# Cyan4973/FiniteStateEntropy

Hardware: NVIDIA H100
Metric: encode+decode GB/s (uncompressed) per GPU on 32 KB blocks; bit-exact vs ref (higher is better)
Workload: dtype u8

## Files before the change

finitestateentropy_b200/csrc/huf_decode.cu:

```cuda
#include "common.cuh"
#include "launchers.h"
#include "huf_dev.cuh"
#include "launch_util.cuh"
#include <cstdlib>
#include <type_traits>

namespace fseb {
namespace hufd {

#ifndef FSEB200_HUFD_HEAD
#define FSEB200_HUFD_HEAD 1
#endif

constexpr int G = 64;
constexpr int THREADS = 4 * G;
constexpr int NWARPS = THREADS / 32;
constexpr int RW = 8;
constexpr u32 RING_BYTES = RW * THREADS * 4;
__host__ __device__ constexpr int threads_for(int ns) { return ns * G; }
__host__ __device__ constexpr u32 ring_bytes(int ns) { return RW * threads_for(ns) * 4; }
constexpr u32 NOERR = 0xFFFFFFFFu;
constexpr unsigned FULL = 0xFFFFFFFFu;
constexpr u32 MIN_ROWS = 160;
constexpr u32 PARK_RANKEND = 128, PARK_LISTSTART = 142;
constexpr u64 HDR_STREAM_MAX = 1ull << 20;

struct __align__(16) Facts {
    u32 bid[G];
    u32 status[G];
    u32 hsize[G];
    u16 dOff[G];
    u16 cut[G];
    u8  tlog[G];
    u8  mbits[G];
    u8  kind[G];
    u8  hard[G];
};
template <int NW>
struct BuildScratchT {
    u8  weights[NW][256];
    u8  sorted[NW][256];
    u32 rankStats[NW][HUF_MAX_TLOG + 1];
    u16 rankRun[NW][HUF_MAX_TLOG + 2];
    u16 rankEnd[NW][HUF_MAX_TLOG + 2];
    u16 listStart[NW][HUF_MAX_TLOG + 2];
};
typedef BuildScratchT<NWARPS> BuildScratch;
static_assert(sizeof(BuildScratch) <= RING_BYTES, "build scratch must fit in the ring");
static_assert(sizeof(BuildScratchT<threads_for(1) / 32>) <= ring_bytes(1), "build scratch must fit in the 1X ring");
static_assert(sizeof(Facts) == 1280, "Facts layout");
constexpr u32 NOBLOCK = 0xFFFFFFFFu;

constexpr u32 STAGE_WARP_BYTES = 32 * 32;
__host__ __device__ constexpr u32 smem_bytes(u32 rows, bool staged, int ns = 4)
{
    return rows * (G * 2) + ring_bytes(ns) + (u32)sizeof(Facts) + (staged ? (u32)(threads_for(ns) / 32) * STAGE_WARP_BYTES : 0u);
}

__device__ __forceinline__ u32 lds_u16(u32 addr) { u16 v; asm volatile("ld.shared.u16 %0, [%1];" : "=h"(v) : "r"(addr)); return v; }
__device__ __forceinline__ u32 lds_u32(u32 addr) { u32 v; asm volatile("ld.shared.u32 %0, [%1];" : "=r"(v) : "r"(addr)); return v; }
__device__ __forceinline__ void sts_u32(u32 addr, u32 v) { asm volatile("st.shared.u32 [%0], %1;" :: "r"(addr), "r"(v) : "memory"); }

__device__ __forceinline__ u32 head_symbols(const u8* outp) { return (u32)(0ull - reinterpret_cast<u64>(outp)) & 31u; }

__device__ __forceinline__ u32 canon_cell(const u16* rankEnd, const u16* listStart, const u8* sorted, u32 idx, u32 tl)
{
    u32 w = 1;
    while (idx >= rankEnd[w]) w++;
    u32 const first = (w == 1) ? 0u : rankEnd[w - 1];
    u32 const k = listStart[w] + ((idx - first) >> (w - 1));
    return (tl + 1 - w) | ((u32)sorted[k] << 8);
}

__device__ u64 warp_huf_read_stats(u8* weights, u32* rankStats, u32* nbSymPtr, u32* tlPtr, const u8* in, u64 srcSize, unsigned lane)
{
    if (!srcSize) return err(E_SRC_WRONG);
    u64 iSize = in[0], oSize;
    if (iSize >= 128) {
        oSize = iSize - 127;
        iSize = (oSize + 1) / 2;
        if (iSize + 1 > srcSize) return err(E_SRC_WRONG);
        if (oSize >= 256) return err(E_CORRUPT);
        for (u32 k = lane; k < (u32)iSize; k += 32) { u8 const v = in[1 + k]; weights[2 * k] = v >> 4; weights[2 * k + 1] = v & 15; }
    } else {
        if (iSize + 1 > srcSize) return err(E_SRC_WRONG);
        oSize = 0;
        if (lane == 0) oSize = d_huf_read_weights_fse(weights, 256, in, iSize);
        oSize = __shfl_sync(FULL, oSize, 0);
        if (is_err(oSize)) return oSize;
    }
    if (lane <= HUF_MAX_TLOG) rankStats[lane] = 0;
    __syncwarp();
    u32 total = 0; bool bad = false;
    for (u32 n = lane; n < (u32)oSize; n += 32) {
        u32 const w = weights[n];
        if (w >= HUF_MAX_TLOG) bad = true;
        else { atomicAdd(&rankStats[w], 1u); total += (1u << w) >> 1; }
    }
    if (__any_sync(FULL, bad)) return err(E_CORRUPT);
    #pragma unroll
    for (int d = 16; d; d >>= 1) total += __shfl_xor_sync(FULL, total, d);
    if (total == 0) return err(E_CORRUPT);
    u32 const tl = hibit(total) + 1;
    if (tl > HUF_MAX_TLOG) return err(E_CORRUPT);
    u32 const rest = (1u << tl) - total;
    u32 const lastW = hibit(rest) + 1;
    if ((1u << hibit(rest)) != rest) return err(E_CORRUPT);
    __syncwarp();
    if (lane == 0) { weights[oSize] = (u8)lastW; rankStats[lastW]++; }
    __syncwarp();
    if ((rankStats[1] < 2) || (rankStats[1] & 1)) return err(E_CORRUPT);
    *tlPtr = tl;
    *nbSymPtr = (u32)(oSize + 1);
    return iSize + 1;
}

template <bool EXT = false, class BS>
__device__ void setup_block(u16* tbl, Facts& fx, BS& bs, u32 rows, int blk, const u8* csrc, u64 csize, int warp)
{
    unsigned const lane = lane_id();
    u8* const weights = bs.weights[warp];
    u8* const sorted = bs.sorted[warp];
    u16* const rankEnd = bs.rankEnd[warp];
    u16* const listStart = bs.listStart[warp];
    u32 nbSym = 0, tl = 0, M = 0, cut = 0, nRows = 0;
    u64 h = warp_huf_read_stats(weights, bs.rankStats[warp], &nbSym, &tl, csrc, csize, lane);
    if (lane == 0) {
        if (!is_err(h) && tl > HUF_MAX_TLOG) h = err(E_TLOG_TOO_LARGE);
        if (!EXT && !is_err(h) && h >= csize) h = err(E_SRC_WRONG);
        if (!is_err(h)) {
            u32 acc = 0, pos = 0;
            rankEnd[0] = 0; listStart[0] = 0;
            for (u32 w = 1; w <= tl; w++) {
                listStart[w] = (u16)pos; bs.rankRun[warp][w] = (u16)pos;
                pos += bs.rankStats[warp][w];
                acc += bs.rankStats[warp][w] << (w - 1);
                rankEnd[w] = (u16)(acc > 0xFFFF ? 0xFFFF : acc);
            }
            rankEnd[tl] = (u16)(1u << tl);
            rankEnd[tl + 1] = 0xFFFF;
            M = tl; cut = 0; nRows = 1u << tl;
            for (u32 m = (tl > 10 ? 10 : tl - 1); m >= 4 && m < tl; m--) {
                u32 const g = 1u << (tl - m);
                u32 const T = rankEnd[tl - m];
                u32 const c = (T + g - 1) & ~(g - 1);
                u32 const r = c + (1u << m) - (c >> (tl - m));
                if (r < nRows) { nRows = r; M = m; cut = c; }
            }
            fx.hard[blk] = (u8)(nRows > rows);
            fx.tlog[blk] = (u8)tl;
            fx.mbits[blk] = (u8)M;
            fx.cut[blk] = (u16)cut;
            fx.dOff[blk] = (u16)(M < tl ? cut - (cut >> (tl - M)) : 0);
            fx.hsize[blk] = EXT ? 0u : (u32)h;
        } else {
            atomicMin(&fx.status[blk], (u32)(0u << 8 | (u32)(0 - h)));
        }
    }
    h = __shfl_sync(FULL, h, 0);
    if (is_err(h)) return;
    M = __shfl_sync(FULL, M, 0); cut = __shfl_sync(FULL, cut, 0); nRows = __shfl_sync(FULL, nRows, 0);
    __syncwarp();
    for (u32 base = 0; base < nbSym; base += 32) {
        u32 const s = base + lane;
        u32 const w = (s < nbSym) ? weights[s] : 0u;
        u32 const peers = __match_any_sync(FULL, w);
        if (w) sorted[bs.rankRun[warp][w] + __popc(peers & ((1u << lane) - 1))] = (u8)s;
        __syncwarp();
        if (w && (peers >> lane) == 1u) bs.rankRun[warp][w] = (u16)(bs.rankRun[warp][w] + __popc(peers));
        __syncwarp();
    }
    u16* const col = tbl + blk;
    if (nRows <= rows) {
        u32 const D = (M < tl) ? cut - (cut >> (tl - M)) : 0u;
        for (u32 row = lane; row < nRows; row += 32) {
            u32 const x = (row < cut || M == tl) ? row : ((row - D) << (tl - M));
            col[row * G] = (u16)canon_cell(rankEnd, listStart, sorted, x, tl);
        }
    } else {
        for (u32 r = lane; r < 128; r += 32) col[r * G] = (u16)(sorted[2 * r] | (sorted[2 * r + 1] << 8));
        if (lane < HUF_MAX_TLOG + 2) { col[(PARK_RANKEND + lane) * G] = rankEnd[lane]; col[(PARK_LISTSTART + lane) * G] = listStart[lane]; }
    }
    __syncwarp();
}

template <bool PASS_A, class Geo, int NS>
__global__ void __launch_bounds__(NS * G, NS == 4 ? 4 : 5)
huf_decode_kernel(Geo g, u8* __restrict__ dst, const u8* __restrict__ cbuf, const u64* __restrict__ csizes,
                  u64* __restrict__ results, const u8* __restrict__ orig, u32 flags, u32 gEff, u32 rows,
                  const u32* __restrict__ list, const u32* __restrict__ listCount, u32* __restrict__ deferList, u32* __restrict__ deferCount)
{
    static_assert(NS == 4 || NS == 1, "4X or 1X");
    constexpr int NT = threads_for(NS);
    constexpr int NW = NT / 32;
    constexpr u32 RB = ring_bytes(NS);
    extern __shared__ __align__(16) unsigned char smem_raw[];
    unsigned char* const ringRaw = smem_raw;
    BuildScratchT<NW>& bs = *reinterpret_cast<BuildScratchT<NW>*>(ringRaw);
    Facts& fx = *reinterpret_cast<Facts*>(ringRaw + RB);
    u16* const tbl = reinterpret_cast<u16*>(smem_raw + RB + sizeof(Facts));
    int const tid = threadIdx.x, warp = tid >> 5, lane = tid & 31;
    u32 const blk0 = blockIdx.x * gEff;
    u32 const nWork = list ? *listCount : g.nBlocks;
    if (blk0 >= nWork) return;
    u32 const blkEnd = min(blk0 + gEff, nWork);

    if (tid < G) { fx.bid[tid] = (blk0 + tid < blkEnd) ? (list ? list[blk0 + tid] : blk0 + tid) : NOBLOCK; fx.status[tid] = NOERR; fx.kind[tid] = 3; fx.hsize[tid] = 0; fx.tlog[tid] = 0; fx.mbits[tid] = 0; fx.cut[tid] = 0; fx.dOff[tid] = 0; fx.hard[tid] = 0; }
    __syncthreads();

    for (int j = warp; j < G; j += NW) {
        u32 const b = fx.bid[j];
        if (b == NOBLOCK) continue;
        u64 const n = dec_len(g, b);
        u64 const cs = dec_csize(g, csizes, b);
        int kind;
        if constexpr (std::is_same_v<Geo, HeaderDescs>) {
            if (n > HUF_BLOCK_MAX) { kind = 3; if (lane == 0) dec_out(g, results, b) = err(E_SRC_WRONG); }
            else kind = 0;
        } else if constexpr (!Geo::DESCS) {
            if (flags & 1u) kind = 0;
            else if (is_err(cs)) { kind = 3; if (lane == 0) results[b] = cs; }
            else if (cs == 0) { kind = orig ? 1 : 3; if (lane == 0) results[b] = orig ? n : 0; }
            else if (n == 0) { kind = 3; if (lane == 0) results[b] = err(E_DST_TOO_SMALL); }
            else if (cs > n) { kind = 3; if (lane == 0) results[b] = err(E_CORRUPT); }
            else if (cs == n) kind = 1;
            else if (cs == 1) kind = 2;
            else kind = 0;
        } else {
            if (n == 0) { kind = 3; if (lane == 0) dec_out(g, results, b) = err(E_DST_TOO_SMALL); }
            else if (n > HUF_BLOCK_MAX) { kind = 3; if (lane == 0) dec_out(g, results, b) = err(E_SRC_WRONG); }
            else if (cs > n) { kind = 3; if (lane == 0) dec_out(g, results, b) = err(E_CORRUPT); }
            else if (cs == n) kind = 1;
            else if (cs == 1) kind = 2;
            else kind = 0;
        }
        if (lane == 0) fx.kind[j] = (u8)kind;
        if (kind == 0) {
            if constexpr (std::is_same_v<Geo, HeaderDescs>) {
                u64 const hb = g.hdrSize[b];
                if (hb) setup_block<true>(tbl, fx, bs, rows, j, g.hdr[b], hb, warp);
                else setup_block(tbl, fx, bs, rows, j, dec_src(g, cbuf, b), cs, warp);
            } else setup_block(tbl, fx, bs, rows, j, dec_src(g, cbuf, b), cs, warp);
            if (deferList && fx.hard[j] && fx.status[j] == NOERR) {
                if (lane == 0) { deferList[atomicAdd(deferCount, 1u)] = b; fx.kind[j] = 3; }
            }
        }
    }
    __syncthreads();

    int const col = 2 * lane + (NS == 4 ? warp >> 2 : warp);
    int const strm = (NS == 4) ? warp & 3 : 0;
    u32 const b = fx.bid[col];
    bool const live = (b != NOBLOCK) && fx.kind[col] == 0 && fx.status[col] == NOERR;
    u32 const n = live ? dec_len(g, b) : 0;
    u32 const seg = (NS == 4) ? (n + 3) / 4 : n;
    u32 segLen = 0;
    u8* outp = (Geo::DESCS && !live) ? nullptr : dec_dst(g, dst, b) + (u64)strm * seg;
    const u8* blockStart = nullptr;
    u64 chunkTop = 0;
    u32 expectBits = 0;
    u32 c0 = 0;
    u32 const tl = fx.tlog[col];

    if (live) {
        const u8* const cs0 = dec_src(g, cbuf, b);
        u64 const cs = dec_csize(g, csizes, b);
        blockStart = cs0;
        const u8* const pay = cs0 + fx.hsize[col];
        u64 const psize = cs - fx.hsize[col];
        u32 code = 0;
        constexpr bool HDR = std::is_same_v<Geo, HeaderDescs>;
        bool tooLong = false;
        if constexpr (NS == 4) {
            if (psize < 10) code = E_CORRUPT;
            else if (3 * seg > n) code = E_CORRUPT;
            else {
                u32 const l1 = rd16(pay), l2 = rd16(pay + 2), l3 = rd16(pay + 4);
                if ((u64)l1 + l2 + l3 + 6 > psize) code = E_CORRUPT;
                else {
                    u32 const l4 = (u32)(psize - 6 - l1 - l2 - l3);
                    u32 const off = 6 + (strm > 0 ? l1 : 0) + (strm > 1 ? l2 : 0) + (strm > 2 ? l3 : 0);
                    u32 const len = strm == 0 ? l1 : strm == 1 ? l2 : strm == 2 ? l3 : l4;
                    u64 const len64 = (HDR && strm == 3) ? psize - 6 - l1 - l2 - l3 : len;
                    if (HDR ? len64 < 1 : len < 1) code = E_SRC_WRONG;
                    else {
                        u8 const last = HDR ? pay[off + len64 - 1] : pay[off + len - 1];
                        if (last == 0) code = (HDR ? len64 >= 8 : len >= 8) ? E_GENERIC : E_CORRUPT;
                        else if (HDR && len64 > HDR_STREAM_MAX) tooLong = true;
                        else {
                            u64 const sBegin = (u64)(pay + off);
                            u64 const e = sBegin + len;
                            chunkTop = ((e - 1) & ~31ull) + 32;
                            c0 = (u32)(8 * (chunkTop - e)) + (8 - hibit(last));
                            expectBits = (u32)(8 * (chunkTop - sBegin));
                            segLen = (strm < 3) ? seg : n - 3 * seg;
                        }
                    }
                }
            }
        } else if (HDR && (psize < 1 || psize > HDR_STREAM_MAX)) {
            if (psize < 1) code = E_SRC_WRONG;
            else if (pay[psize - 1] == 0) code = E_GENERIC;
            else tooLong = true;
        } else {
            u32 const len = (u32)psize;
            u8 const last = pay[len - 1];
            if (last == 0) code = (len >= 8) ? E_GENERIC : E_CORRUPT;
            else {
                u64 const sBegin = (u64)pay;
                u64 const e = sBegin + len;
                chunkTop = ((e - 1) & ~31ull) + 32;
                c0 = (u32)(8 * (chunkTop - e)) + (8 - hibit(last));
                expectBits = (u32)(8 * (chunkTop - sBegin));
                segLen = n;
            }
        }
        if (code) atomicMin(&fx.status[col], (u32)((1u + strm) << 8 | code));
        if (tooLong) atomicMin(&fx.status[col], (u32)(5u << 8 | E_CORRUPT));
    }
    __syncthreads();
    bool const go = live && fx.status[col] == NOERR;
    if (!go) segLen = 0;

    u32 const ringLane = (u32)__cvta_generic_to_shared(ringRaw) + tid * 4;
    u32 pLimit;
    if constexpr (Geo::DESCS) pLimit = go ? (u32)((chunkTop - dec_floor(g, cbuf, blockStart)) >> 5) - 1u : 0u;
    else pLimit = go ? (u32)((chunkTop - (reinterpret_cast<u64>(cbuf) & ~31ull)) >> 5) - 1u : 0u;
    u32 m0 = 0, m1 = 0, m2 = 0, m3 = 0, m4 = 0, m5 = 0, m6 = 0, m7 = 0;
    constexpr bool staged = PASS_A;
    auto load_pair = [&](u32 pr) {
        u64 const a = chunkTop - 32ull * (min(pr, pLimit) + 1);
        if (!staged) {
            asm volatile("ld.global.nc.v4.b32 {%0, %1, %2, %3}, [%8];\n\t"
                         "ld.global.nc.v4.b32 {%4, %5, %6, %7}, [%8+16];"
                         : "=r"(m0), "=r"(m1), "=r"(m2), "=r"(m3), "=r"(m4), "=r"(m5), "=r"(m6), "=r"(m7) : "l"(a));
            asm volatile("prefetch.global.L2 [%0];" :: "l"(chunkTop - 32ull * (min(pr + 2, pLimit) + 1)));
            return;
        }
        u32 const dead = (a & 127) == 0;
        asm volatile("{\n\t.reg .pred p;\n\t.reg .b64 pol;\n\tsetp.ne.u32 p, %9, 0;\n\t"
                     "createpolicy.fractional.L2::evict_first.b64 pol, 1.0;\n\t"
                     "@p ld.global.nc.L2::cache_hint.v4.b32 {%0, %1, %2, %3}, [%8], pol;\n\t"
                     "@p ld.global.nc.L2::cache_hint.v4.b32 {%4, %5, %6, %7}, [%8+16], pol;\n\t"
                     "@!p ld.global.nc.v4.b32 {%0, %1, %2, %3}, [%8];\n\t"
                     "@!p ld.global.nc.v4.b32 {%4, %5, %6, %7}, [%8+16];\n\t}"
                     : "=r"(m0), "=r"(m1), "=r"(m2), "=r"(m3), "=r"(m4), "=r"(m5), "=r"(m6), "=r"(m7) : "l"(a), "r"(dead));
        {
            if ((a & 127) == 96 && pr + 11 <= pLimit) asm volatile("cp.async.bulk.prefetch.L2.global [%0], 128;" :: "l"(a - 352));
        }
    };

    u32 w0 = 0, w1 = 0, w2 = 0, r = 0;
    u32 kBase = 0;
    u32 q = 0;
    auto store_next = [&]() {
        u32 const a = ringLane + (q & 1) * (4 * NT * 4);
        bool const lowHalf = (q & 1) != 0;
        sts_u32(a, lowHalf ? m3 : m7); sts_u32(a + NT * 4, lowHalf ? m2 : m6);
        sts_u32(a + 2 * NT * 4, lowHalf ? m1 : m5); sts_u32(a + 3 * NT * 4, lowHalf ? m0 : m4);
        q++;
        if (!(q & 1)) load_pair(q >> 1);
    };
    auto unread = [&]() -> u32 { return 4 * q - kBase - (r >> 5); };
    auto top_up = [&](u32 threshold) { if (unread() <= threshold) store_next(); };

    if (go) {
        u32 const k0 = c0 >> 5;
        r = c0 & 31;
        q = 2 * (k0 >> 3);
        load_pair(q >> 1);
        store_next(); store_next();
        kBase = k0;
        auto fetch_word = [&]() -> u32 {
            u32 const v = lds_u32(ringLane + (kBase & 7) * (NT * 4));
            kBase++;
            if (!(kBase & 7)) store_next();
            return v;
        };
        w0 = fetch_word(); w1 = fetch_word(); w2 = fetch_word();
        top_up(4);
    }

    u32 const tblCol = (u32)__cvta_generic_to_shared(tbl) + col * 2;
    u32 const M = fx.mbits[col];
    u32 const shX = 32 - (tl ? tl : 1);
    u32 const shY = 32 - (M ? M : 1);
    int const dOff = (int)fx.dOff[col];
    u32 const tblColD = tblCol + (u32)dOff * (G * 2);
    bool const hardBlk = fx.hard[col] != 0;

    static_assert(NT * 4 % 32 == 0 && (NT * 4 & (NT * 4 - 1)) == 0, "slot stride: a power of two, a multiple of 32");
    u32 const tid4 = tid * 4;
    u32 const ringBase = (u32)__cvta_generic_to_shared(ringRaw);
    u32 const slotBias = kBase * (NT * 4);
    u32 hi = __funnelshift_l(w1, w0, r), lo = __funnelshift_l(w2, w1, r);
#define HUFD_LOOKUP(E, H) do { \
        int const a_ = (int)((H) >> shX) - dOff; \
        int const y_ = (int)((H) >> shY); \
        E = lds_u16((u32)min(a_, y_) * (G * 2) + tblColD); \
    } while (0)
#define HUFD_ADVANCE(PACKED) do { \
        u32 const rOld_ = r; \
        r = __dp4a((u32)(PACKED), 0x00010001u, r); \
        u32 const ra_ = ((rOld_ * (NT * 4 / 32u) + slotBias) & ((RW - 1) * NT * 4)) | tid4; \
        asm volatile("{\n\t.reg .pred p;\n\t.reg .b32 t;\n\t" \
                     "xor.b32 t, %4, %5;\n\tand.b32 t, t, 32;\n\tsetp.ne.u32 p, t, 0;\n\t" \
                     "@p mov.b32 %0, %1;\n\t@p mov.b32 %1, %2;\n\t@p ld.shared.u32 %2, [%3];\n\t}" \
                     : "+r"(w0), "+r"(w1), "+r"(w2) : "r"(ringBase + ra_), "r"(r), "r"(rOld_) : "memory"); \
        hi = __funnelshift_l(w1, w0, r); lo = __funnelshift_l(w2, w1, r); \
    } while (0)

    u32 pos = 0;
    constexpr bool withHead = Geo::DESCS && FSEB200_HUFD_HEAD;
    bool const fastOk = withHead ? go && !hardBlk && segLen >= head_symbols(outp) + 32u
                                 : go && !hardBlk && ((reinterpret_cast<u64>(outp) & 31) == 0);
    u32 const headN = (withHead && fastOk) ? head_symbols(outp) : 0u;
    if constexpr (withHead) {
        for (u32 i = 0; i < headN; i++) {
            if ((i & 7) == 0) top_up(4);
            u32 e;
            HUFD_LOOKUP(e, hi);
            HUFD_ADVANCE(e);
            outp[pos++] = (u8)(e >> 8);
        }
    }
    u32 const nIter = fastOk ? (segLen - headN) >> 5 : 0u;
    u32 const nIterW = __reduce_max_sync(FULL, nIter);
    u32 const stageW = (u32)__cvta_generic_to_shared(tbl) + rows * (G * 2) + (u32)warp * STAGE_WARP_BYTES;
    for (u32 it = 0; it < nIterW; it++) {
        bool const act = it < nIter;
        u32 o[8];
        if (act) {
            #pragma unroll
            for (int h = 0; h < 8; h++) {
                if ((h & 3) == 0) top_up(4);
                else if ((h & 3) == 2 && __builtin_expect(__any_sync(__activemask(), unread() <= 3), 0)) top_up(3);
                u32 e0, e1, e2, e3, hi1;
                HUFD_LOOKUP(e0, hi); hi1 = __funnelshift_l(lo, hi, e0); HUFD_LOOKUP(e1, hi1);
                u32 const p01 = e0 | (e1 << 16);
                HUFD_ADVANCE(p01);
                HUFD_LOOKUP(e2, hi); hi1 = __funnelshift_l(lo, hi, e2); HUFD_LOOKUP(e3, hi1);
                u32 const p23 = e2 | (e3 << 16);
                HUFD_ADVANCE(p23);
                o[h] = __byte_perm(p01, p23, 0x7531);
            }
        }
        if (!staged) {
            if (act)
                asm volatile("st.global.v4.b32 [%0], {%1, %2, %3, %4};\n\tst.global.v4.b32 [%0+16], {%5, %6, %7, %8};"
                             :: "l"(outp + pos), "r"(o[0]), "r"(o[1]), "r"(o[2]), "r"(o[3]), "r"(o[4]), "r"(o[5]), "r"(o[6]), "r"(o[7]) : "memory");
            if (act) pos += 32;
            continue;
        }
        if (act)
            asm volatile("st.shared.v4.b32 [%0], {%1, %2, %3, %4};\n\tst.shared.v4.b32 [%0+16], {%5, %6, %7, %8};"
                         :: "r"(stageW + (u32)lane * 32), "r"(o[0]), "r"(o[1]), "r"(o[2]), "r"(o[3]), "r"(o[4]), "r"(o[5]), "r"(o[6]), "r"(o[7]) : "memory");
        __syncwarp();
        u64 const dstHere = reinterpret_cast<u64>(outp + pos);
        u32 const o32 = (u32)dstHere - pos;
        bool const lineDone = ((((o32 + pos) | 127u) + 1u) - o32) <= headN + nIter * 32u;
        u32 const flags = (act ? 1u : 0u) | (lineDone ? 2u : 0u);
        #pragma unroll
        for (int k = 0; k < 2; k++) {
            int const src = k * 16 + (lane >> 1);
            u32 const half = (u32)(lane & 1) * 16;
            u64 const q = __shfl_sync(FULL, dstHere, src);
            u32 const srcFlags = __shfl_sync(FULL, flags, src);
            u32 x0, x1, x2, x3;
            asm volatile("ld.shared.v4.b32 {%0, %1, %2, %3}, [%4];" : "=r"(x0), "=r"(x1), "=r"(x2), "=r"(x3) : "r"(stageW + (u32)src * 32 + half));
            u32 const keep = (srcFlags & 2u) && ((q + half) & 127) < 96;
            if (srcFlags & 1u)
                asm volatile("{\n\t.reg .pred p;\n\t.reg .b64 pl, pf;\n\tsetp.ne.u32 p, %5, 0;\n\t"
                             "createpolicy.fractional.L2::evict_last.b64 pl, 1.0;\n\t"
                             "createpolicy.fractional.L2::evict_first.b64 pf, 1.0;\n\t"
                             "@p st.global.L2::cache_hint.v4.b32 [%0], {%1, %2, %3, %4}, pl;\n\t"
                             "@!p st.global.L2::cache_hint.v4.b32 [%0], {%1, %2, %3, %4}, pf;\n\t}"
                             :: "l"(q + half), "r"(x0), "r"(x1), "r"(x2), "r"(x3), "r"(keep) : "memory");
        }
        __syncwarp();
        if (act) pos += 32;
    }
    if (pos < segLen) {
        const u16* const colp = tbl + col;
        auto parked_cell = [&](u32 idx) -> u32 {
            u32 w = 1;
            while (idx >= colp[(PARK_RANKEND + w) * G]) w++;
            u32 const first = (w == 1) ? 0u : colp[(PARK_RANKEND + w - 1) * G];
            u32 const k = colp[(PARK_LISTSTART + w) * G] + ((idx - first) >> (w - 1));
            return (tl + 1 - w) | (((colp[(k >> 1) * G] >> (8 * (k & 1))) & 0xFFu) << 8);
        };
        u32 cnt = 0;
        while (pos < segLen) {
            if ((cnt++ & 7) == 0) top_up(4);
            u32 e;
            if (hardBlk) e = parked_cell(hi >> (32 - tl));
            else HUFD_LOOKUP(e, hi);
            HUFD_ADVANCE(e);
            outp[pos++] = (u8)(e >> 8);
        }
    }
#undef HUFD_LOOKUP
#undef HUFD_ADVANCE

    if (go) {
        u64 const fetched = 4ull * q - unread();
        u64 const consumed = 32ull * (fetched - 3) + (r & 31);
        if (consumed != (u64)expectBits) atomicMin(&fx.status[col], (u32)(5u << 8 | E_CORRUPT));
    }
    __syncthreads();
    if (tid < G) {
        u32 const bb = fx.bid[tid];
        if (bb != NOBLOCK && fx.kind[tid] == 0) {
            u32 const st = fx.status[tid];
            u64 rv = (st == NOERR) ? (u64)dec_len(g, bb) : err(st & 0xFF);
            if ((st >> 8) == 5u && ((flags & 2u) || (!(flags & 1u) && d_huf_select_decoder(dec_len(g, bb), dec_csize(g, csizes, bb))))) rv = HUF_X2_PENDING;
            dec_out(g, results, bb) = rv;
        }
    }
    for (int j = 0; j < G; j++) {
        int const kd = fx.kind[j];
        if (kd != 1 && kd != 2) continue;
        u32 const bb = fx.bid[j];
        u32 const nn = dec_len(g, bb);
        u64 const cs = dec_csize(g, csizes, bb);
        u8* const o = dec_dst(g, dst, bb);
        if (kd == 2) { u8 const v = dec_src(g, cbuf, bb)[0]; for (u32 i = tid; i < nn; i += NT) o[i] = v; }
        else {
            const u8* const s = (cs == 0) ? dec_orig(g, orig, bb) : dec_src(g, cbuf, bb);
            for (u32 i = tid; i < nn; i += NT) o[i] = s[i];
        }
        if (tid == 0) dec_out(g, results, bb) = nn;
    }
}

constexpr int FORM_THREADS = 256;
struct HufMixedSplit {
    const u64* dstCap; const u8* single; u64* cap4; u64* cap1; const u64* res1; u64* result;
    u32 nBlocks;
};

__global__ void __launch_bounds__(FORM_THREADS) huf_mixed_split_kernel(HufMixedSplit g)
{
    u64 const b = (u64)blockIdx.x * FORM_THREADS + threadIdx.x;
    if (b >= g.nBlocks) return;
    u64 const n = g.dstCap[b], none = (u64)HUF_BLOCK_MAX + 1;
    bool const one = g.single[b] != 0;
    g.cap4[b] = one ? none : n;
    g.cap1[b] = one ? n : none;
}

__global__ void __launch_bounds__(FORM_THREADS) huf_mixed_merge_kernel(HufMixedSplit g)
{
    u64 const b = (u64)blockIdx.x * FORM_THREADS + threadIdx.x;
    if (b >= g.nBlocks) return;
    if (g.single[b]) g.result[b] = g.res1[b];
}

}

namespace {

template <class Geo, int NS>
cudaError_t huf_decode(const Geo& g, void* dst, const void* cbuf, const u64* csizes, u64* results,
                       const void* orig, cudaStream_t stream, u32 flags)
{
    static SmemOptIn optinA, optinB;
    static u32 const reqA = [] { const char* e = std::getenv("FSEB200_HUFD_ROWS"); return e ? (u32)std::atoi(e) : 306u; }();
    static u32 const reqB = [] { const char* e = std::getenv("FSEB200_HUFD_ROWS_B"); return e ? (u32)std::atoi(e) : 808u; }();
    if (g.nBlocks == 0) return cudaSuccess;
    int const dev = current_device();
    u32 const optin = (u32)device_smem_optin(dev);
    auto fit = [optin](bool staged) { u32 const fixed = hufd::smem_bytes(0, staged, NS); return optin > fixed ? (optin - fixed) / (hufd::G * 2) : 0u; };
    u32 const rowsA = max(hufd::MIN_ROWS, min(reqA, fit(true)));
    u32 const rowsB = min(reqB, fit(false));
    size_t const smemA = hufd::smem_bytes(rowsA, true, NS);
    bool const twoPass = rowsB > rowsA;
    cudaError_t e = optinA.ensure(hufd::huf_decode_kernel<true, Geo, NS>, dev, (int)smemA);
    if (e == cudaSuccess && twoPass) e = optinB.ensure(hufd::huf_decode_kernel<false, Geo, NS>, dev, (int)hufd::smem_bytes(rowsB, false, NS));
    if (e != cudaSuccess) return e;
    u32* scratch = nullptr;
    if (twoPass) {
        scratch = (u32*)stream_scratch(1, stream, ((size_t)g.nBlocks + 1) * sizeof(u32), &e);
        if (e != cudaSuccess) return e;
        e = cudaMemsetAsync(scratch, 0, sizeof(u32), stream);
        if (e != cudaSuccess) return e;
    }
    int perSm = 0;
    if (cudaOccupancyMaxActiveBlocksPerMultiprocessor(&perSm, hufd::huf_decode_kernel<true, Geo, NS>, hufd::threads_for(NS), smemA) != cudaSuccess || perSm < 1) perSm = 1;
    u32 const slots = (u32)perSm * (u32)device_sm_count(dev);
    u32 gEff = (u32)hufd::G;
    if ((u64)g.nBlocks * 5 > (u64)slots * hufd::G * 4) {
        u32 const rounds = (g.nBlocks + slots * hufd::G - 1) / (slots * hufd::G);
        gEff = (g.nBlocks + slots * rounds - 1) / (slots * rounds);
        if (gEff > (u32)hufd::G) gEff = hufd::G;
        if (gEff < 1) gEff = 1;
    }
    unsigned const grid = (g.nBlocks + gEff - 1) / gEff;
    hufd::huf_decode_kernel<true, Geo, NS><<<grid, hufd::threads_for(NS), smemA, stream>>>(g, (u8*)dst, (const u8*)cbuf, csizes, results, (const u8*)orig, flags, gEff, rowsA,
                                                                    nullptr, nullptr, twoPass ? scratch + 1 : nullptr, scratch);
    e = cudaGetLastError();
    if (e != cudaSuccess) return e;
    if (twoPass) {
        unsigned const gridB = (g.nBlocks + hufd::G - 1) / hufd::G;
        hufd::huf_decode_kernel<false, Geo, NS><<<gridB, hufd::threads_for(NS), hufd::smem_bytes(rowsB, false, NS), stream>>>(g, (u8*)dst, (const u8*)cbuf, csizes, results, (const u8*)orig, flags,
                                                                                            (u32)hufd::G, rowsB, scratch + 1, scratch, nullptr, nullptr);
        e = cudaGetLastError();
        if (e != cudaSuccess) return e;
    }
    if (flags == 1u) return cudaSuccess;
    if constexpr (Geo::DESCS) return launch_huf_x2_fixup_blocks(g, NS, stream);
    else return launch_huf_x2_fixup(g, dst, cbuf, csizes, results, stream);
}
}

cudaError_t launch_huf_decode(const BatchGeom& g, void* dst, const void* cbuf, const u64* csizes, u64* results,
                              const void* orig, cudaStream_t stream, u32 flags)
{
    return huf_decode<BatchGeom, 4>(g, dst, cbuf, csizes, results, orig, stream, flags);
}

cudaError_t launch_huf_decode_blocks(const BlockDescs& g, int nStreams, cudaStream_t stream)
{
    return nStreams == 1 ? huf_decode<BlockDescs, 1>(g, nullptr, nullptr, nullptr, nullptr, nullptr, stream, 0u)
                         : huf_decode<BlockDescs, 4>(g, nullptr, nullptr, nullptr, nullptr, nullptr, stream, 0u);
}

cudaError_t launch_huf_decode_headers(const HeaderDescs& g, int nStreams, cudaStream_t stream, const u8* single)
{
    if (nStreams == 1) return huf_decode<HeaderDescs, 1>(g, nullptr, nullptr, nullptr, nullptr, nullptr, stream, 1u);
    if (nStreams) return huf_decode<HeaderDescs, 4>(g, nullptr, nullptr, nullptr, nullptr, nullptr, stream, 1u);
    if (g.nBlocks == 0) return cudaSuccess;
    size_t const n = g.nBlocks;
    cudaError_t e;
    u64* const s = (u64*)stream_scratch(13, stream, 3 * sizeof(u64) * n, &e);
    if (e != cudaSuccess) return e;
    hufd::HufMixedSplit m;
    m.dstCap = g.dstCap; m.single = single; m.cap4 = s; m.cap1 = s + n; m.res1 = s + 2 * n; m.result = g.result; m.nBlocks = g.nBlocks;
    unsigned const grid = (unsigned)((n + hufd::FORM_THREADS - 1) / hufd::FORM_THREADS);
    hufd::huf_mixed_split_kernel<<<grid, hufd::FORM_THREADS, 0, stream>>>(m);
    if ((e = cudaGetLastError()) != cudaSuccess) return e;
    HeaderDescs d = g;
    d.dstCap = m.cap4;
    if ((e = huf_decode<HeaderDescs, 4>(d, nullptr, nullptr, nullptr, nullptr, nullptr, stream, 1u)) != cudaSuccess) return e;
    d.dstCap = m.cap1; d.result = s + 2 * n;
    if ((e = huf_decode<HeaderDescs, 1>(d, nullptr, nullptr, nullptr, nullptr, nullptr, stream, 1u)) != cudaSuccess) return e;
    hufd::huf_mixed_merge_kernel<<<grid, hufd::FORM_THREADS, 0, stream>>>(m);
    return cudaGetLastError();
}

}
```

Baseline: 415.2.

## Decode FSE-compressed Huffman weights in parallel across lanes before table setup

Before, each warp decoded each block's FSE-compressed weight header serially on lane 0 while the other 31 lanes waited, one block at a time. Now every lane of a warp decodes the header of a different column block up front, writing the weights to a per-block global scratch area. The per-block setup then only copies the decoded weights back into shared memory. This adds a global scratch buffer plus extra global traffic, and pass B indexes that scratch by its own blockIdx, which may not match the layout pass A used.

```diff
diff --git a/finitestateentropy_b200/csrc/huf_decode.cu b/finitestateentropy_b200/csrc/huf_decode.cu
--- a/finitestateentropy_b200/csrc/huf_decode.cu
+++ b/finitestateentropy_b200/csrc/huf_decode.cu
@@ -72,7 +72,8 @@
     return (tl + 1 - w) | ((u32)sorted[k] << 8);
 }
 
-__device__ u64 warp_huf_read_stats(u8* weights, u32* rankStats, u32* nbSymPtr, u32* tlPtr, const u8* in, u64 srcSize, unsigned lane)
+__device__ u64 warp_huf_read_stats(u8* weights, u32* rankStats, u32* nbSymPtr, u32* tlPtr, const u8* in, u64 srcSize, unsigned lane,
+                                   u64 fseW, const u8* fseOut)
 {
     if (!srcSize) return err(E_SRC_WRONG);
     u64 iSize = in[0], oSize;
@@ -84,10 +85,9 @@
         for (u32 k = lane; k < (u32)iSize; k += 32) { u8 const v = in[1 + k]; weights[2 * k] = v >> 4; weights[2 * k + 1] = v & 15; }
     } else {
         if (iSize + 1 > srcSize) return err(E_SRC_WRONG);
-        oSize = 0;
-        if (lane == 0) oSize = d_huf_read_weights_fse(weights, 256, in, iSize);
-        oSize = __shfl_sync(FULL, oSize, 0);
+        oSize = fseW;
         if (is_err(oSize)) return oSize;
+        for (u32 k = lane; k < (u32)oSize; k += 32) weights[k] = fseOut[k];
     }
     if (lane <= HUF_MAX_TLOG) rankStats[lane] = 0;
     __syncwarp();
@@ -116,7 +116,7 @@
 }
 
 template <bool EXT = false, class BS>
-__device__ void setup_block(u16* tbl, Facts& fx, BS& bs, u32 rows, int blk, const u8* csrc, u64 csize, int warp)
+__device__ void setup_block(u16* tbl, Facts& fx, BS& bs, u32 rows, int blk, const u8* csrc, u64 csize, int warp, u64 fseW, const u8* fseOut)
 {
     unsigned const lane = lane_id();
     u8* const weights = bs.weights[warp];
@@ -124,7 +124,7 @@
     u16* const rankEnd = bs.rankEnd[warp];
     u16* const listStart = bs.listStart[warp];
     u32 nbSym = 0, tl = 0, M = 0, cut = 0, nRows = 0;
-    u64 h = warp_huf_read_stats(weights, bs.rankStats[warp], &nbSym, &tl, csrc, csize, lane);
+    u64 h = warp_huf_read_stats(weights, bs.rankStats[warp], &nbSym, &tl, csrc, csize, lane, fseW, fseOut);
     if (lane == 0) {
         if (!is_err(h) && tl > HUF_MAX_TLOG) h = err(E_TLOG_TOO_LARGE);
         if (!EXT && !is_err(h) && h >= csize) h = err(E_SRC_WRONG);
@@ -184,11 +184,50 @@
     __syncwarp();
 }
 
+template <class Geo>
+__device__ __forceinline__ int block_kind(const Geo& g, const u64* csizes, const u8* orig, u32 flags, u32 b, u64& verdict)
+{
+    u64 const n = dec_len(g, b);
+    u64 const cs = dec_csize(g, csizes, b);
+    verdict = 0;
+    if constexpr (std::is_same_v<Geo, HeaderDescs>) {
+        if (n > HUF_BLOCK_MAX) { verdict = err(E_SRC_WRONG); return 3; }
+        return 0;
+    } else if constexpr (!Geo::DESCS) {
+        if (flags & 1u) return 0;
+        if (is_err(cs)) { verdict = cs; return 3; }
+        if (cs == 0) { verdict = orig ? n : 0; return orig ? 1 : 3; }
+        if (n == 0) { verdict = err(E_DST_TOO_SMALL); return 3; }
+        if (cs > n) { verdict = err(E_CORRUPT); return 3; }
+        if (cs == n) return 1;
+        if (cs == 1) return 2;
+        return 0;
+    } else {
+        if (n == 0) { verdict = err(E_DST_TOO_SMALL); return 3; }
+        if (n > HUF_BLOCK_MAX) { verdict = err(E_SRC_WRONG); return 3; }
+        if (cs > n) { verdict = err(E_CORRUPT); return 3; }
+        if (cs == n) return 1;
+        if (cs == 1) return 2;
+        return 0;
+    }
+}
+
+template <class Geo>
+__device__ __forceinline__ void block_header(const Geo& g, const u8* cbuf, const u64* csizes, u32 b, const u8*& in, u64& sz)
+{
+    if constexpr (std::is_same_v<Geo, HeaderDescs>) {
+        u64 const hb = g.hdrSize[b];
+        if (hb) { in = g.hdr[b]; sz = hb; return; }
+    }
+    in = dec_src(g, cbuf, b); sz = dec_csize(g, csizes, b);
+}
+
 template <bool PASS_A, class Geo, int NS>
 __global__ void __launch_bounds__(NS * G, NS == 4 ? 4 : 5)
 huf_decode_kernel(Geo g, u8* __restrict__ dst, const u8* __restrict__ cbuf, const u64* __restrict__ csizes,
                   u64* __restrict__ results, const u8* __restrict__ orig, u32 flags, u32 gEff, u32 rows,
-                  const u32* __restrict__ list, const u32* __restrict__ listCount, u32* __restrict__ deferList, u32* __restrict__ deferCount)
+                  const u32* __restrict__ list, const u32* __restrict__ listCount, u32* __restrict__ deferList, u32* __restrict__ deferCount,
+                  u8* fseScratch)
 {
     static_assert(NS == 4 || NS == 1, "4X or 1X");
     constexpr int NT = threads_for(NS);
@@ -208,39 +247,35 @@
     if (tid < G) { fx.bid[tid] = (blk0 + tid < blkEnd) ? (list ? list[blk0 + tid] : blk0 + tid) : NOBLOCK; fx.status[tid] = NOERR; fx.kind[tid] = 3; fx.hsize[tid] = 0; fx.tlog[tid] = 0; fx.mbits[tid] = 0; fx.cut[tid] = 0; fx.dOff[tid] = 0; fx.hard[tid] = 0; }
     __syncthreads();
 
-    for (int j = warp; j < G; j += NW) {
+    constexpr int COLS = G / NW;
+    u8* const fseOut = fseScratch + ((u64)blockIdx.x * G + warp) * 256;
+    u64 fseW = 0;
+    if (lane < COLS) {
+        u32 const b = fx.bid[warp + lane * NW];
+        u64 verdict;
+        if (b != NOBLOCK && block_kind(g, csizes, orig, flags, b, verdict) == 0) {
+            const u8* in; u64 sz;
+            block_header(g, cbuf, csizes, b, in, sz);
+            if (sz && in[0] < 128 && (u64)in[0] + 1 <= sz) fseW = d_huf_read_weights_fse(fseOut + (u64)lane * NW * 256, 256, in, in[0]);
+        }
+    }
+    __syncwarp();
+    for (int k = 0; k < COLS; k++) {
+        int const j = warp + k * NW;
+        u64 const fw = __shfl_sync(FULL, fseW, k);
         u32 const b = fx.bid[j];
         if (b == NOBLOCK) continue;
-        u64 const n = dec_len(g, b);
-        u64 const cs = dec_csize(g, csizes, b);
-        int kind;
-        if constexpr (std::is_same_v<Geo, HeaderDescs>) {
-            if (n > HUF_BLOCK_MAX) { kind = 3; if (lane == 0) dec_out(g, results, b) = err(E_SRC_WRONG); }
-            else kind = 0;
-        } else if constexpr (!Geo::DESCS) {
-            if (flags & 1u) kind = 0;
-            else if (is_err(cs)) { kind = 3; if (lane == 0) results[b] = cs; }
-            else if (cs == 0) { kind = orig ? 1 : 3; if (lane == 0) results[b] = orig ? n : 0; }
-            else if (n == 0) { kind = 3; if (lane == 0) results[b] = err(E_DST_TOO_SMALL); }
-            else if (cs > n) { kind = 3; if (lane == 0) results[b] = err(E_CORRUPT); }
-            else if (cs == n) kind = 1;
-            else if (cs == 1) kind = 2;
-            else kind = 0;
-        } else {
-            if (n == 0) { kind = 3; if (lane == 0) dec_out(g, results, b) = err(E_DST_TOO_SMALL); }
-            else if (n > HUF_BLOCK_MAX) { kind = 3; if (lane == 0) dec_out(g, results, b) = err(E_SRC_WRONG); }
-            else if (cs > n) { kind = 3; if (lane == 0) dec_out(g, results, b) = err(E_CORRUPT); }
-            else if (cs == n) kind = 1;
-            else if (cs == 1) kind = 2;
-            else kind = 0;
-        }
+        u64 verdict;
+        int const kind = block_kind(g, csizes, orig, flags, b, verdict);
+        if (kind == 3 && lane == 0) dec_out(g, results, b) = verdict;
         if (lane == 0) fx.kind[j] = (u8)kind;
         if (kind == 0) {
+            const u8* const fo = fseOut + (u64)k * NW * 256;
             if constexpr (std::is_same_v<Geo, HeaderDescs>) {
                 u64 const hb = g.hdrSize[b];
-                if (hb) setup_block<true>(tbl, fx, bs, rows, j, g.hdr[b], hb, warp);
-                else setup_block(tbl, fx, bs, rows, j, dec_src(g, cbuf, b), cs, warp);
-            } else setup_block(tbl, fx, bs, rows, j, dec_src(g, cbuf, b), cs, warp);
+                if (hb) setup_block<true>(tbl, fx, bs, rows, j, g.hdr[b], hb, warp, fw, fo);
+                else setup_block(tbl, fx, bs, rows, j, dec_src(g, cbuf, b), dec_csize(g, csizes, b), warp, fw, fo);
+            } else setup_block(tbl, fx, bs, rows, j, dec_src(g, cbuf, b), dec_csize(g, csizes, b), warp, fw, fo);
             if (deferList && fx.hard[j] && fx.status[j] == NOERR) {
                 if (lane == 0) { deferList[atomicAdd(deferCount, 1u)] = b; fx.kind[j] = 3; }
             }
@@ -596,14 +631,16 @@
         if (gEff < 1) gEff = 1;
     }
     unsigned const grid = (g.nBlocks + gEff - 1) / gEff;
+    u8* const fseScratch = (u8*)stream_scratch(14, stream, (size_t)grid * hufd::G * 256, &e);
+    if (e != cudaSuccess) return e;
     hufd::huf_decode_kernel<true, Geo, NS><<<grid, hufd::threads_for(NS), smemA, stream>>>(g, (u8*)dst, (const u8*)cbuf, csizes, results, (const u8*)orig, flags, gEff, rowsA,
-                                                                    nullptr, nullptr, twoPass ? scratch + 1 : nullptr, scratch);
+                                                                    nullptr, nullptr, twoPass ? scratch + 1 : nullptr, scratch, fseScratch);
     e = cudaGetLastError();
     if (e != cudaSuccess) return e;
     if (twoPass) {
         unsigned const gridB = (g.nBlocks + hufd::G - 1) / hufd::G;
         hufd::huf_decode_kernel<false, Geo, NS><<<gridB, hufd::threads_for(NS), hufd::smem_bytes(rowsB, false, NS), stream>>>(g, (u8*)dst, (const u8*)cbuf, csizes, results, (const u8*)orig, flags,
-                                                                                            (u32)hufd::G, rowsB, scratch + 1, scratch, nullptr, nullptr);
+                                                                                            (u32)hufd::G, rowsB, scratch + 1, scratch, nullptr, nullptr, fseScratch);
         e = cudaGetLastError();
         if (e != cudaSuccess) return e;
     }
```

After: 415.5, median of 6. About the same (+0.1%).
